# apple/ml-unigen

Measured on AMD Instinct MI355X. Metric: train-step samples/s (1.5B, 256^2 img), higher is better.
Workload: dtype bf16

## Files before the change

include/unigen_hip.h:

```cpp
#ifndef UNIGEN_HIP_H
#define UNIGEN_HIP_H

#include <stdint.h>
#include <hip/hip_runtime_api.h>

#ifdef __cplusplus
extern "C" {
#endif

#define UG_ABI_VERSION 7

const char* ug_last_error(void);
int ug_abi_version(void);

typedef struct ug_handle ug_handle;
int ug_create(ug_handle** out);
int ug_destroy(ug_handle* h);

#define UG_EPI_BF16 0
#define UG_EPI_F32 1
#define UG_EPI_RESID 2
int ug_gemm_bf16(const ug_handle* h, const void* A, int64_t lda, int a_kmajor, const void* B, int64_t ldb, int b_kmajor,
                 void* C, int64_t ldc, int64_t M, int64_t N, int64_t K, int epilogue, const void* bias,
                 const float* resid, int64_t ldr, int beta, const float* alpha_dev, int policy, hipStream_t stream);
// ... 42 lines not shown
#define UG_MASK_I64 2
#define UG_MASK_BOOL 3
int ug_attn_mask_compress(const void* mask, int mask_dtype, int64_t stride_b, int64_t stride_row,
                          uint64_t* bits, uint8_t* tileany, int64_t B, int64_t L, int* err_flag,
                          hipStream_t stream);
int ug_attn_mask_causal(const uint8_t* key_valid , uint64_t* bits, uint8_t* tileany,
                        int64_t B, int64_t L, hipStream_t stream);
int ug_attn_fwd(const void* q, const void* k, const void* v, int64_t ldq, void* o,
                int64_t ldo, float* lse, const uint64_t* bits, const uint8_t* tileany, int64_t B, int64_t L,
                int64_t Lp, int H, int HKV, int head_dim, float scale, hipStream_t stream);
int ug_attn_bwd(const void* q, const void* k, const void* v, int64_t ldq,
                const void* o, const void* dout, int64_t ldo, const float* lse,
                float* delta, void* dq, void* dk, void* dv, int64_t ldg, const uint64_t* bits,
                const uint8_t* tileany, int64_t B, int64_t L, int64_t Lp, int H, int HKV, int head_dim,
                float scale, float* dkv_ws, const float* rope_cos, const float* rope_sin, float* dbias_qkv, hipStream_t stream);

int ug_kv_store(const void* qkv, int64_t ldq, int64_t k_col, int64_t v_col, void* cache_k, void* cache_v,
                int64_t rows, int64_t L, int HKV, int head_dim, int64_t Tmax, const int* pos_dev, int pos_host,
                hipStream_t stream);
int ug_rope_at(void* qkv, const float* cos_tab, const float* sin_tab, int64_t rows, int64_t ldq, int nheads,
               int head_dim, const int* pos_dev, int64_t max_pos, hipStream_t stream);
int ug_attn_decode(const void* q, int64_t ldq, const void* cache_k, const void* cache_v, const uint8_t* key_valid,
                   void* o, int64_t ldo, int64_t rows, int H, int HKV, int head_dim, int64_t Tmax,
                   const int* len_dev, float scale, hipStream_t stream);
int ug_gemv_bf16(const void* x, int64_t ldx, int64_t R, const void* W, int64_t ldw, float* acc, int64_t acc_stride_r,
                 int64_t acc_stride_n, int64_t N, int64_t K, hipStream_t stream);
int ug_decode_finish_resid_norm(float* acc, int64_t ldacc, float* x, const float* w, void* xn, int64_t rows, int64_t cols,
                                float eps, int* pos_inc, int* len_inc, hipStream_t stream);
int ug_decode_gemv(const void* x, int64_t ldx, int64_t R, const void* W, int64_t ldw, float* acc, int64_t ldacc, int64_t N,
                   int64_t K, float* zero0, int64_t n0, float* zero1, int64_t n1, float* ss_zero, hipStream_t stream);
// ... 170 lines not shown
```

ml-unigen_amd/csrc/attention.hip:

```cpp
#include "common.h"
#include "unigen_hip.h"
#include "vmem_asm.h"
#include <stdlib.h>

namespace {

constexpr int HD = 128;
constexpr int RM_LD = 144;
constexpr int RM_BYTES = 64 * RM_LD * 2;
typedef __attribute__((ext_vector_type(4))) short s16x4_t;

template <typename T> __device__ __forceinline__ bool mask_attend(T v, int* err);
template <> __device__ __forceinline__ bool mask_attend<float>(float v, int* err) {
  if (v == 0.f) return true;
  if (!(v <= -1e9f) && err) atomicOr(err, 2);
  return false;
}
template <> __device__ __forceinline__ bool mask_attend<bf16_t>(bf16_t v, int* err) { return mask_attend<float>(bf2f(v), err); }
template <> __device__ __forceinline__ bool mask_attend<int64_t>(int64_t v, int* err) {
  if (v == 0) return true;
  if (v > -1000000000LL && err) atomicOr(err, 2);
  return false;
}
template <> __device__ __forceinline__ bool mask_attend<uint8_t>(uint8_t v, int*) { return v != 0; }
// ... 151 lines not shown

struct AttnArgs {
  const bf16_t* q; const bf16_t* k; const bf16_t* v;
  bf16_t* o; const bf16_t* dout;
  bf16_t* dq; bf16_t* dk; bf16_t* dv;
  float* dkv_ws;
  float* lse; const float* delta;
  const uint64_t* bits; const uint8_t* tileany;
  int64_t ldq, ldo, ldg;
  int B, L, Lp, nW, H, HKV;
  float scale;
  const float* rope_cos; const float* rope_sin; float* dbias;
  int order;
  int dkv_heads;
  int ablate;
};

__device__ __forceinline__ void rope_bwd_pair(float& g1, float& g2, float c, float s) {
#pragma clang fp contract(off)
  const float x1 = bf2f(f2bf(g1)), x2 = bf2f(f2bf(g2));
  const float a1 = x1 * c, a2 = x2 * c;
  const float b1 = x2 * s, b2 = x1 * s;
  g1 = a1 + b1; g2 = a2 - b2;
}
template <int N>
__device__ __forceinline__ void halve_sum(float (&x)[64], int lane, int m) {
  const bool up = (lane & m) != 0;
#pragma unroll
  for (int i = 0; i < N / 2; ++i) {
    const float lo = x[i], hi = x[i + N / 2];
// ... 748 lines not shown
  return ((row & 3) << 2) | ((0x78 >> (m * 2)) & 3);
}
__device__ __forceinline__ bf16x8_t frag16(const char* tile, int rb, int ks, int lane) {
  const int row = rb * 16 + (lane & 15);
  return *reinterpret_cast<const bf16x8_t*>(tile + row * 256 + (((ks * 4 + (lane >> 4)) ^ swz16b(row)) << 4));
}
__device__ __forceinline__ bf16x8_t frag16_tr(const char* tile, int rb, int jp, int lane) {
  const int i16 = lane & 15, g = lane >> 4;
  const int row = jp * 32 + g * 4 + (i16 >> 2);
  const char* p0 = tile + row * 256 + (((rb * 2 + ((i16 & 3) >> 1)) ^ swz16b(row)) << 4) + (i16 & 1) * 8;
  const s16x4_t lo = __builtin_amdgcn_ds_read_tr16_b64_v4i16((__attribute__((address_space(3))) s16x4_t*)p0);
  const s16x4_t hi = __builtin_amdgcn_ds_read_tr16_b64_v4i16((__attribute__((address_space(3))) s16x4_t*)(p0 + 16 * 256));
  return __builtin_shufflevector(lo, hi, 0, 1, 2, 3, 4, 5, 6, 7);
}

__global__ __launch_bounds__(256, 2) void attn_bwd_dkv_dma_kernel(AttnArgs p) {
  __shared__ __attribute__((aligned(16))) char ring[2 * 2 * T32_BYTES];
  __shared__ __attribute__((aligned(16))) float lse_s[2][64], dl_s[2][64];
  __shared__ __attribute__((aligned(16))) uint64_t word_s[2][64];
  const int tid = threadIdx.x, lane = tid & 63, g = lane >> 4;
  const int wave = __builtin_amdgcn_readfirstlane(tid >> 6);
  const int grp = p.H / p.HKV;
  const int HPW = p.dkv_heads;
  const WgCoord wc = wg_coord((int)blockIdx.x, p.nW, p.H / HPW, p.HKV, p.B, false, p.order != 0);
  if (!wc.ok) return;
  const int t = wc.tile, b = wc.b, h0 = wc.h * HPW, hk = h0 / grp;
  const int krow = t * 64 + wave * 16 + (lane & 15);
  const int krow_c = min(krow, p.L - 1);
  const bf16_t* kseq = p.k + (int64_t)b * p.L * p.ldq + hk * HD;
  const bf16_t* vseq = p.v + (int64_t)b * p.L * p.ldq + hk * HD;
// ... 56 lines not shown
  bool r_in = false;
  auto fetch_rows = [&](int qt) {
    const int qr = qt * 64 + lane;
    const int qc = min(qr, p.L - 1);
    r_lse = p.lse[((int64_t)b * p.H + h) * p.L + qc];
    r_dl = p.delta[((int64_t)b * p.H + h) * p.L + qc];
    r_word = p.bits[((int64_t)b * p.L + qc) * p.nW + t];
    r_in = qr < p.L;
  };

  int qt = next_visible(0);
  int hleft = qt < p.nW ? HPW - 1 : 0;
  if (qt < p.nW) { stage(qt, 0); if (wave == 0) fetch_rows(qt); }
#pragma unroll
  for (int ks = 0; ks < 4; ++ks) { tie(kf[ks]); tie(vf[ks]); }
  for (int it = 0; qt < p.nW; ++it) {
    int qn = next_visible(qt + 1);
    const int slot = it & 1;
    wait_vm<0>();
    if (wave == 0) {
      tie(r_lse); tie(r_dl); tie(r_word);
      lse_s[slot][lane] = r_lse * 1.4426950408889634f;
      dl_s[slot][lane] = r_dl * p.scale;
      word_s[slot][lane] = r_in ? r_word : 0ull;
    }
    asm volatile("s_waitcnt lgkmcnt(0)" ::: "memory");
    asm volatile("s_barrier" ::: "memory");
    if (qn >= p.nW && hleft > 0) {
      --hleft; ++h;
      qseq += HD; doseq += HD;
      qn = next_visible(0);
    }
    if (qn < p.nW) { stage(qn, slot ^ 1); if (wave == 0) fetch_rows(qn); }
// ... 9 lines not shown
        dp = __builtin_amdgcn_mfma_f32_16x16x32_bf16(frag16(Ds, j, ks, lane), vf[ks], dp, 0, 0, 0);
      }
      const f32x4_t ls = *reinterpret_cast<const f32x4_t*>(&lse_s[slot][j * 16 + g * 4]);
      const f32x4_t dl4 = *reinterpret_cast<const f32x4_t*>(&dl_s[slot][j * 16 + g * 4]);
#pragma unroll
      for (int r = 0; r < 4; ++r) {
        const int ql = j * 16 + g * 4 + r;
        const bool on = (word_s[slot][ql] >> kbit) & 1ull;
        const float e = on ? __builtin_amdgcn_exp2f(__builtin_fmaf(sc[r], c1, -ls[r])) : 0.f;
        pr[j][r] = e;
        ds[j][r] = e * __builtin_fmaf(dp[r], p.scale, -dl4[r]);
      }
    }
    const bf16x8_t pf0 = pack_p(pr[0], pr[1]), pf1 = pack_p(pr[2], pr[3]);
    const bf16x8_t sf0 = pack_p(ds[0], ds[1]), sf1 = pack_p(ds[2], ds[3]);
#pragma unroll
    for (int d = 0; d < 8; ++d) {
      dvt[d] = __builtin_amdgcn_mfma_f32_16x16x32_bf16(frag16_tr(Ds, d, 0, lane), pf0, dvt[d], 0, 0, 0);
      dkt[d] = __builtin_amdgcn_mfma_f32_16x16x32_bf16(frag16_tr(Qs, d, 0, lane), sf0, dkt[d], 0, 0, 0);
    }
#pragma unroll
    for (int d = 0; d < 8; ++d) {
      dvt[d] = __builtin_amdgcn_mfma_f32_16x16x32_bf16(frag16_tr(Ds, d, 1, lane), pf1, dvt[d], 0, 0, 0);
      dkt[d] = __builtin_amdgcn_mfma_f32_16x16x32_bf16(frag16_tr(Qs, d, 1, lane), sf1, dkt[d], 0, 0, 0);
    }
    qt = qn;
  }
  __syncthreads();
  float* tw = reinterpret_cast<float*>(ring) + wave * (16 * 132);
  const int ldws = 2 * p.HKV * HD;
// ... 4 lines not shown
#pragma unroll
      for (int r = 0; r < 4; ++r) tw[(lane & 15) * 132 + d * 16 + g * 4 + r] = pass == 0 ? dkt[d][r] : dvt[d][r];
    __builtin_amdgcn_wave_barrier();
    asm volatile("s_waitcnt lgkmcnt(0)" ::: "memory");
#pragma unroll
    for (int i = 0; i < 16; ++i) {
      const int kr = t * 64 + wave * 16 + i;
      if (kr < p.L) {
        float* dst = p.dkv_ws + ((int64_t)b * p.L + kr) * ldws + (pass * p.HKV + hk) * HD;
        atomicAdd(dst + lane, tw[i * 132 + lane]);
        atomicAdd(dst + 64 + lane, tw[i * 132 + 64 + lane]);
      }
    }
    __builtin_amdgcn_wave_barrier();
    asm volatile("s_waitcnt lgkmcnt(0)" ::: "memory");
  }
}

__global__ __launch_bounds__(256) void dkv_finish_rope_kernel(float* __restrict__ ws, bf16_t* __restrict__ dk, bf16_t* __restrict__ dv,
                                                              int64_t ldg, int64_t tokens, int L, int HKV,
                                                              const float* __restrict__ cs, const float* __restrict__ sn,
                                                              float* __restrict__ dbias_k, float* __restrict__ dbias_v,
                                                              int rows_per_block) {
  __shared__ float red[256 * 16];
  const int per_row = HKV * 16;
  const int slot = threadIdx.x / per_row, nslots = 256 / per_row;
  const int hk = (threadIdx.x % per_row) >> 4, c4 = threadIdx.x & 15;
  const int kvw = HKV * HD;
  float sum[16];
#pragma unroll
// ... 67 lines not shown
    float4* src = reinterpret_cast<float4*>(ws + row * 2 * kvw + c);
    const float4 v = *src;
    *src = make_float4(0.f, 0.f, 0.f, 0.f);
    uint2 w; w.x = pack_bf2(v.x, v.y); w.y = pack_bf2(v.z, v.w);
    bf16_t* dst = c < kvw ? dk + row * ldg + c : dv + row * ldg + (c - kvw);
    *reinterpret_cast<uint2*>(dst) = w;
  }
}

int check_common(const char* fn, int64_t B, int64_t L, int64_t Lp, int H, int HKV, int hd, int64_t ldq) {
  UG_REQUIRE(B > 0 && L > 0, "%s: empty batch", fn);
  UG_REQUIRE(hd == HD, "%s: head_dim %d unsupported (this build is specialised for 128)", fn, hd);
  UG_REQUIRE(H % HKV == 0, "%s: H=%d not a multiple of HKV=%d", fn, H, HKV);
  UG_REQUIRE(Lp % 64 == 0 && Lp >= L, "%s: Lp=%ld must be a multiple of 64 and >= L", fn, (long)Lp);
  UG_REQUIRE(ldq % 8 == 0, "%s: row stride must be a multiple of 8 elements", fn);
  return UG_OK;
}

}

extern "C" int ug_attn_mask_compress(const void* mask, int mask_dtype, int64_t stride_b, int64_t stride_row,
                                     uint64_t* bits, uint8_t* tileany, int64_t B, int64_t L, int* err_flag,
                                     hipStream_t st) {
  UG_REQUIRE(B > 0 && L > 0 && mask && bits && tileany, "ug_attn_mask_compress: bad args");
  const int nW = (int)((L + 63) / 64);
  const int64_t nwaves = B * L * nW;
  dim3 grid((unsigned)((nwaves + 3) / 4)), block(256);
  switch (mask_dtype) {
    case UG_MASK_F32: hipLaunchKernelGGL(mask_compress_kernel<float>, grid, block, 0, st, (const float*)mask, stride_b, stride_row, bits, (int)B, (int)L, nW, err_flag); break;
    case UG_MASK_BF16: hipLaunchKernelGGL(mask_compress_kernel<bf16_t>, grid, block, 0, st, (const bf16_t*)mask, stride_b, stride_row, bits, (int)B, (int)L, nW, err_flag); break;
// ... 70 lines not shown
  if (int rc = check_common("ug_attn_bwd", B, L, Lp, H, HKV, head_dim, ldq)) return rc;
  UG_REQUIRE((rope_cos == nullptr) == (rope_sin == nullptr) && (!rope_cos || (ug_aligned16(rope_cos) && ug_aligned16(rope_sin))),
             "ug_attn_bwd: rope_cos / rope_sin come together, 16-byte aligned");
  UG_REQUIRE(ug_aligned16(dkv_ws), "ug_attn_bwd: workspace alignment");
  UG_REQUIRE(ug_aligned16(q) && ug_aligned16(k) && ug_aligned16(v) && ug_aligned16(dout) && ldo % 8 == 0 && ldg % 4 == 0,
             "ug_attn_bwd: alignment");
  AttnArgs a{};
  a.q = (const bf16_t*)q; a.k = (const bf16_t*)k; a.v = (const bf16_t*)v;
  a.dout = (const bf16_t*)dout; a.lse = const_cast<float*>(lse); a.delta = delta;
  a.o = const_cast<bf16_t*>((const bf16_t*)o);
  a.dq = (bf16_t*)dq; a.dk = (bf16_t*)dk; a.dv = (bf16_t*)dv; a.dkv_ws = dkv_ws;
  a.bits = bits; a.tileany = tileany;
  a.ldq = ldq; a.ldo = ldo; a.ldg = ldg; a.B = (int)B; a.L = (int)L; a.Lp = (int)Lp; a.nW = (int)((L + 63) / 64);
  a.H = H; a.HKV = HKV; a.scale = scale;
  { static const int abl = [] { const char* e = getenv("UNIGEN_ATTN_ABLATE"); return e ? atoi(e) : 0; }(); a.ablate = abl; }
  static const int use32 = [] { const char* e = getenv("UNIGEN_ATTN_DQ32"); return e ? atoi(e) : 1; }();
  static const int fuse = [] { const char* e = getenv("UNIGEN_ATTN_BWD_FUSE_ROPE"); return e ? atoi(e) : 1; }();
  const int64_t tokens = B * L;
  auto rope_pass = [&](void* x, int nheads) -> int { return rope_cos ? ug_rope(x, rope_cos, rope_sin, tokens, L, ldg, nheads, HD, 1, st) : UG_OK; };
  auto colsum_pass = [&](const void* x, float* out, int cols) -> int { return dbias ? ug_colsum_bf16(x, ldg, out, tokens, cols, st) : UG_OK; };
  static const int ord = [] { const char* e = getenv("UNIGEN_ATTN_ORDER"); return e ? atoi(e) : 1; }();
  a.order = (ord >> 1) & 1;
  if (use32 && L >= 256 && L <= 4096 && (int64_t)((L + 127) / 128) * H * B >= 512) {
    if (fuse) { a.rope_cos = rope_cos; a.rope_sin = rope_sin; a.dbias = dbias; }
    hipLaunchKernelGGL(attn_bwd_dq32_kernel<4>, dim3(wg_grid((L + 127) / 128, H, HKV, B)), dim3(256), 0, st, a);
    UG_CHECK_LAUNCH("ug_attn_bwd(dq)");
    if (!fuse) { if (int rc = rope_pass(dq, H)) return rc; if (int rc = colsum_pass(dq, dbias, H * HD)) return rc; }
  } else {
    hipLaunchKernelGGL(attn_bwd_dq_kernel, dim3(wg_grid(a.nW, H, HKV, B)), dim3(256), 0, st, a);
    UG_CHECK_LAUNCH("ug_attn_bwd(dq)");
    if (int rc = rope_pass(dq, H)) return rc;
    if (int rc = colsum_pass(dq, dbias, H * HD)) return rc;
  }
  a.rope_cos = a.rope_sin = nullptr; a.dbias = nullptr;
  float* dbias_k = dbias ? dbias + H * HD : nullptr;
  float* dbias_v = dbias ? dbias + (H + HKV) * HD : nullptr;
  if (dkv_ws) {
    static const int dma = [] { const char* e = getenv("UNIGEN_ATTN_DKV_DMA"); return e ? atoi(e) : 1; }();
    a.order = (ord >> 2) & 1;
    static const int hpw_env = [] { const char* e = getenv("UNIGEN_ATTN_DKV_HEADS"); return e ? atoi(e) : 2; }();
    static const int hpw_min_wgs = [] { const char* e = getenv("UNIGEN_ATTN_DKV_MIN_WGS"); return e ? atoi(e) : 1024; }();
    a.dkv_heads = (hpw_env >= 1 && (H / HKV) % hpw_env == 0 && (int64_t)a.nW * (H / hpw_env) * B >= hpw_min_wgs) ? hpw_env : 1;
    if (dma && L <= 4096) hipLaunchKernelGGL(attn_bwd_dkv_dma_kernel, dim3(wg_grid(a.nW, H / a.dkv_heads, HKV, B)), dim3(256), 0, st, a);
    else hipLaunchKernelGGL(attn_bwd_dkv_kernel<true>, dim3(wg_grid(a.nW, H, HKV, B)), dim3(256), 0, st, a);
    UG_CHECK_LAUNCH("ug_attn_bwd(dkv split)");
    if (fuse && (rope_cos || dbias) && HKV <= 16 && (HKV & (HKV - 1)) == 0) {
      static const int fin_wgs = [] { const char* e = getenv("UNIGEN_ATTN_FINISH_WGS"); return e ? atoi(e) : 128; }();
      const int rpb = (int)((tokens + fin_wgs - 1) / fin_wgs < 8 ? 8 : (tokens + fin_wgs - 1) / fin_wgs);
      hipLaunchKernelGGL(dkv_finish_rope_kernel, dim3((unsigned)((tokens + rpb - 1) / rpb)), dim3(256), 0, st, dkv_ws, a.dk, a.dv, ldg,
                         tokens, (int)L, HKV, rope_cos, rope_sin, dbias_k, dbias_v, rpb);
      UG_CHECK_LAUNCH("ug_attn_bwd(dkv finish + rope)");
      return UG_OK;
    }
    const int64_t total = B * L * (2 * HKV * HD / 4);
    int64_t gsz = (total + 255) / 256; if (gsz > 4096) gsz = 4096;
    hipLaunchKernelGGL(dkv_finish_kernel, dim3((unsigned)gsz), dim3(256), 0, st, dkv_ws, a.dk, a.dv, ldg, B * L, HKV * HD);
    UG_CHECK_LAUNCH("ug_attn_bwd(dkv finish)");
  } else {
    hipLaunchKernelGGL(attn_bwd_dkv_kernel<false>, dim3(wg_grid(a.nW, HKV, HKV, B)), dim3(256), 0, st, a);
    UG_CHECK_LAUNCH("ug_attn_bwd(dkv)");
  }
  if (int rc = rope_pass(dk, HKV)) return rc;
  if (int rc = colsum_pass(dk, dbias_k, HKV * HD)) return rc;
  if (int rc = colsum_pass(dv, dbias_v, HKV * HD)) return rc;
  return UG_OK;
}
```

ml-unigen_amd/unigen_hip/lib.py:

```python
import ctypes
import os
import subprocess

_HERE = os.path.dirname(os.path.abspath(__file__))
CSRC_DIR = os.path.normpath(os.path.join(_HERE, "..", "csrc"))
LIB_PATH = os.environ.get("UNIGEN_HIP_LIB") or os.path.join(CSRC_DIR, "libunigen_hip.so")

ABI_VERSION = 7
P = ctypes.c_void_p
I64 = ctypes.c_int64
I32 = ctypes.c_int
F32 = ctypes.c_float

SIGNATURES = {
    "ug_abi_version": [],
    "ug_create": [P],
    "ug_destroy": [P],
    "ug_gemm_bf16": [P, P, I64, I32, P, I64, I32, P, I64, I64, I64, I64, I32, P, P, I64, I32, P, I32, P],
    "ug_gemm_bf16_qkv_rope": [P, P, I64, P, I64, P, P, I64, I64, I64, I64, P, P, I64, I64, I32, P],
    "ug_gemm_bf16_swiglu_bwd": [P, P, I64, P, I64, P, I64, P, I64, I64, I64, I64, P],
    "ug_gemm_bf16_swiglu": [P, P, I64, P, I64, P, I64, P, I64, I64, I64, I64, P],
    "ug_cast_f32_bf16": [P, P, I64, P],
    "ug_rmsnorm_fwd": [P, P, P, P, I64, I64, F32, I32, P],
    "ug_rmsnorm_bwd": [P, P, P, P, P, P, P, I64, I64, P],
    "ug_rope": [P, P, P, I64, I64, I64, I32, I32, I32, P],
    "ug_swiglu_fwd": [P, P, I64, I64, P],
    "ug_swiglu_bwd": [P, P, P, I64, I64, P],
    "ug_gelu": [P, P, P, I64, P],
    "ug_embed_fwd": [P, P, P, I64, I64, I64, P, P],
    "ug_embed_bwd": [P, P, P, I64, I64, I64, P],
    "ug_embed_bwd_sorted": [P, P, P, P, I64, I64, I64, F32, P],
    "ug_gather_rows_bf16": [P, I64, P, P, I64, I64, I64, I32, P],
    "ug_colsum_bf16": [P, I64, P, I64, I64, P],
    "ug_attn_mask_compress": [P, I32, I64, I64, P, P, I64, I64, P, P],
    "ug_attn_mask_causal": [P, P, P, I64, I64, P],
    "ug_attn_fwd": [P, P, P, I64, P, I64, P, P, P, I64, I64, I64, I32, I32, I32, F32, P],
    "ug_attn_bwd": [P, P, P, I64, P, P, I64, P, P, P, P, P, I64, P, P, I64, I64, I64, I32, I32, I32, F32, P, P, P, P, P],
    "ug_kv_store": [P, I64, I64, I64, P, P, I64, I64, I32, I32, I64, P, I32, P],
    "ug_rope_at": [P, P, P, I64, I64, I32, I32, P, I64, P],
    "ug_attn_decode": [P, I64, P, P, P, P, I64, I64, I32, I32, I32, I64, P, F32, P],
    "ug_gemv_bf16": [P, I64, I64, P, I64, P, I64, I64, I64, I64, P],
    "ug_decode_gemv": [P, I64, I64, P, I64, P, I64, I64, I64, P, I64, P, I64, P, P],
    "ug_decode_gemv_resid_norm": [P, P, I64, P, P, P, I64, P, I64, P, I64, I64, I64, P, I64, P, I64, P, P],
    "ug_decode_gemv_swiglu": [P, I64, P, F32, I64, I64, P, I64, P, I64, I64, I64, P, I64, P, I64, P, P],
    "ug_gemm_set_fused_tile_height": [I32],
    "ug_attn_decode_fused": [P, I64, P, F32, I64, P, P, P, P, P, P, P, P, I64, I64, I32, I32, I32, I64, I64, F32, P],
    "ug_decode_finish_resid_norm": [P, I64, P, P, P, I64, I64, F32, P, P, P],
    "ug_decode_sw_supported": [I64, I64, I64, I32],
    "ug_decode_sw_kblock": [P, I64, I64, P, I64, P, I64, I64, I64, P, I64, P, I64, P, P],
    "ug_decode_sw_resid": [P, I64, I64, P, I64, I64, I64, P, P],
    "ug_decode_sw_gate_up": [P, P, I64, P, P, F32, I64, I64, P, I64, I64, P, I64, P],
    "ug_decode_sw_head": [P, P, I64, P, P, F32, I64, I64, P, I64, I64, P, I64, P, P, P],
# ... 54 lines not shown
    "ug_nchw_to_nhwc": [P, P, I64, I32, I64, I32, P],
    "ug_nhwc_to_nchw": [P, P, I64, I32, I64, I32, P],
    "ug_lfq_pack": [P, I64, P, I64, I32, P],
    "ug_lfq_unpack": [P, P, I64, I32, P, P],
    "ug_probe_layouts": [P, I64, P],
}

_lib = None

PROFILE = None


def family_of(name):
    if name.startswith("ug_gemm_bf16"):
        return "gemm"
    if name in ("ug_attn_fwd", "ug_attn_bwd"):
        return "attention"
    if name.startswith(("ug_conv", "ug_groupnorm", "ug_amax", "ug_lfq", "ug_nchw", "ug_nhwc", "ug_gemm_f32", "ug_softmax_rows", "ug_linear_",
                        "ug_layernorm", "ug_siglip")):
        return "tokenizer_and_towers"
    if name == "ug_adamw_flat":
        return "adamw"
    return "elementwise"


def _profiled(name, fn):
    fam = family_of(name)

    def call(*args):
        prof = PROFILE
        if prof is None:
# ... 67 lines not shown
```

ml-unigen_amd/unigen_hip/ops.py:

```python
import ctypes
import math
import torch

from . import lib as _l

UG_EPI_BF16, UG_EPI_F32, UG_EPI_RESID = 0, 1, 2
_MASK_DTYPES = {torch.float32: 0, torch.bfloat16: 1, torch.int64: 2, torch.bool: 3}


GEMM_PROFILE = None
GEMM_PROFILE_FUSED = None


def _stream():
    return torch.cuda.current_stream().cuda_stream


def _p(t):
    return 0 if t is None else t.data_ptr()


_HANDLES = {}
GEMM_POLICY = -1
UG_GEMM_NARROW_EPILOGUE, UG_GEMM_POLICY_AUTO_BITS = 0x100, 0xff
# ... 407 lines not shown
                                   _p(mb.tileany), B, L, Lp, H, HKV, hd, scale, _stream()), "ug_attn_fwd")
    return o, lse


_DKV_WS = {}


def _dkv_workspace(tokens, width, device):
    key = (device, tokens, width)
    if key not in _DKV_WS:
        _DKV_WS.clear()
        _DKV_WS[key] = torch.zeros((tokens, width), dtype=torch.float32, device=device)
    return _DKV_WS[key]


def attn_bwd(qkv, o, lse, dout, mb, H, HKV, hd, scale=None, split_heads=True, rope=None, dbias=None, out=None):
    B, L, Lp = mb.B, mb.L, mb.Lp
    scale = 1.0 / math.sqrt(hd) if scale is None else scale
    q = qkv[:, : H * hd]
    k = qkv[:, H * hd: (H + HKV) * hd]
    v = qkv[:, (H + HKV) * hd:]
    dqkv = torch.empty_like(qkv) if out is None else out
    dq = dqkv[:, : H * hd]
    dk = dqkv[:, H * hd: (H + HKV) * hd]
    dv = dqkv[:, (H + HKV) * hd:]
    delta = torch.empty((B, H, L), dtype=torch.float32, device=qkv.device)
    ws = _dkv_workspace(B * L, 2 * HKV * hd, qkv.device) if split_heads and H > HKV else None
    _l.check(_l.load().ug_attn_bwd(_p(q), _p(k), _p(v), qkv.stride(0), _p(o), _p(dout), o.stride(0),
                                   _p(lse), _p(delta), _p(dq), _p(dk), _p(dv), dqkv.stride(0), _p(mb.bits),
                                   _p(mb.tileany), B, L, Lp, H, HKV, hd, scale, _p(ws), _p(rope[0] if rope else None),
                                   _p(rope[1] if rope else None), _p(dbias), _stream()), "ug_attn_bwd")
    return dqkv


def kv_store(qkv, cache_k, cache_v, rows, L, H, HKV, hd, Tmax, pos_dev=None, pos_host=0):
    _l.check(_l.load().ug_kv_store(_p(qkv), qkv.stride(0), H * hd, (H + HKV) * hd, _p(cache_k), _p(cache_v), rows, L, HKV, hd,
                                   Tmax, _p(pos_dev), pos_host, _stream()), "ug_kv_store")


def rope_at_(qkv, cos, sin, nheads, hd, pos_dev):
    _l.check(_l.load().ug_rope_at(_p(qkv), _p(cos), _p(sin), qkv.shape[0], qkv.stride(0), nheads, hd, _p(pos_dev),
                                  cos.shape[0], _stream()), "ug_rope_at")
# ... 613 lines not shown
```

Baseline: 130.3.

## Hand off dS from dK/dV kernel to a dQ kernel instead of recomputing

Adds an attention backward route where the dK/dV kernel writes each bf16 dS tile to a global workspace. A new dQ kernel then streams K and dS tiles and does only the dS·K matmul, so it no longer recomputes QK^T, softmax and dP. A separate delta kernel is added, and the route is on by default for eligible GQA shapes. The cost is a workspace of up to 1 GiB (B·H·nW²·8KB) and the extra HBM traffic to write and re-read dS, and the dQ pass now has to run after dK/dV instead of alongside it.

```diff
diff --git a/include/unigen_hip.h b/include/unigen_hip.h
--- a/include/unigen_hip.h
+++ b/include/unigen_hip.h
@@ -80,6 +80,12 @@
                 float* delta, void* dq, void* dk, void* dv, int64_t ldg, const uint64_t* bits,
                 const uint8_t* tileany, int64_t B, int64_t L, int64_t Lp, int H, int HKV, int head_dim,
                 float scale, float* dkv_ws, const float* rope_cos, const float* rope_sin, float* dbias_qkv, hipStream_t stream);
+int ug_attn_bwd_handoff(const void* q, const void* k, const void* v, int64_t ldq,
+                        const void* o, const void* dout, int64_t ldo, const float* lse,
+                        float* delta, void* dq, void* dk, void* dv, int64_t ldg, const uint64_t* bits,
+                        const uint8_t* tileany, int64_t B, int64_t L, int64_t Lp, int H, int HKV, int head_dim,
+                        float scale, float* dkv_ws, const float* rope_cos, const float* rope_sin, float* dbias_qkv,
+                        void* ds_ws, int64_t ds_ws_bytes, int dkv_heads, hipStream_t stream);
 
 int ug_kv_store(const void* qkv, int64_t ldq, int64_t k_col, int64_t v_col, void* cache_k, void* cache_v,
                 int64_t rows, int64_t L, int HKV, int head_dim, int64_t Tmax, const int* pos_dev, int pos_host,
diff --git a/ml-unigen_amd/csrc/attention.hip b/ml-unigen_amd/csrc/attention.hip
--- a/ml-unigen_amd/csrc/attention.hip
+++ b/ml-unigen_amd/csrc/attention.hip
@@ -189,6 +189,8 @@
   int order;
   int dkv_heads;
   int ablate;
+  char* ds_ws;
+  int delta_lanes;
 };
 
 __device__ __forceinline__ void rope_bwd_pair(float& g1, float& g2, float c, float s) {
@@ -967,6 +969,8 @@
   return __builtin_shufflevector(lo, hi, 0, 1, 2, 3, 4, 5, 6, 7);
 }
 
+constexpr int DS_BLOCK = 64 * 64 * 2;
+template <bool HANDOFF>
 __global__ __launch_bounds__(256, 2) void attn_bwd_dkv_dma_kernel(AttnArgs p) {
   __shared__ __attribute__((aligned(16))) char ring[2 * 2 * T32_BYTES];
   __shared__ __attribute__((aligned(16))) float lse_s[2][64], dl_s[2][64];
@@ -1053,9 +1057,11 @@
   if (qt < p.nW) { stage(qt, 0); if (wave == 0) fetch_rows(qt); }
 #pragma unroll
   for (int ks = 0; ks < 4; ++ks) { tie(kf[ks]); tie(vf[ks]); }
+  const uint32_t dsoff = (uint32_t)(wave * 2048 + ((g * 16 + ((lane & 15) ^ (g << 2))) << 4));
   for (int it = 0; qt < p.nW; ++it) {
     int qn = next_visible(qt + 1);
     const int slot = it & 1;
+    const int hcur = h;
     wait_vm<0>();
     if (wave == 0) {
       tie(r_lse); tie(r_dl); tie(r_word);
@@ -1095,6 +1101,11 @@
     }
     const bf16x8_t pf0 = pack_p(pr[0], pr[1]), pf1 = pack_p(pr[2], pr[3]);
     const bf16x8_t sf0 = pack_p(ds[0], ds[1]), sf1 = pack_p(ds[2], ds[3]);
+    if constexpr (HANDOFF) {
+      char* blk = p.ds_ws + ((((int64_t)b * p.H + hcur) * p.nW + qt) * p.nW + t) * DS_BLOCK + dsoff;
+      *reinterpret_cast<bf16x8_t*>(blk) = sf0;
+      *reinterpret_cast<bf16x8_t*>(blk + 1024) = sf1;
+    }
 #pragma unroll
     for (int d = 0; d < 8; ++d) {
       dvt[d] = __builtin_amdgcn_mfma_f32_16x16x32_bf16(frag16_tr(Ds, d, 0, lane), pf0, dvt[d], 0, 0, 0);
@@ -1129,6 +1140,198 @@
     }
     __builtin_amdgcn_wave_barrier();
     asm volatile("s_waitcnt lgkmcnt(0)" ::: "memory");
+  }
+}
+
+
+template <int NP>
+__global__ __launch_bounds__(256) void attn_bwd_delta_kernel(AttnArgs p) {
+  const int64_t idx = (int64_t)blockIdx.x * 256 + threadIdx.x;
+  const int part = (int)(idx % NP);
+  const int64_t rh = idx / NP;
+  const int h = (int)(rh % p.H);
+  const int64_t row = min(rh / p.H, (int64_t)p.B * p.L - 1);
+  const bool in = rh / p.H < (int64_t)p.B * p.L;
+  const bf16_t* orow = p.o + row * p.ldo + h * HD;
+  const bf16_t* drow = p.dout + row * p.ldo + h * HD;
+  float dl = 0.f;
+#pragma unroll
+  for (int ks = 0; ks < 16 / NP; ++ks) {
+    const bf16x8_t dof = *reinterpret_cast<const bf16x8_t*>(drow + (ks * NP + part) * 8);
+    const bf16x8_t of = *reinterpret_cast<const bf16x8_t*>(orow + (ks * NP + part) * 8);
+#pragma unroll
+    for (int e = 0; e < 8; ++e) dl += bf2f((bf16_t)of[e]) * bf2f((bf16_t)dof[e]);
+  }
+  dl += __shfl_xor(dl, 1, 64);
+  if (NP == 4) dl += __shfl_xor(dl, 2, 64);
+  if (part == 0 && in) const_cast<float*>(p.delta)[((row / p.L) * p.H + h) * p.L + row % p.L] = dl;
+}
+
+__global__ __launch_bounds__(256, 2) void attn_bwd_dq_handoff_kernel(AttnArgs p) {
+  __shared__ __attribute__((aligned(16))) char ring[2 * 2 * T32_BYTES];
+  const int tid = threadIdx.x, lane = tid & 63;
+  const int wave = __builtin_amdgcn_readfirstlane(tid >> 6);
+  const int n = lane & 31, hh = lane >> 5, i16 = lane & 15, grp = (lane >> 4) & 1;
+  const WgCoord wc = wg_coord((int)blockIdx.x, (p.L + 127) / 128, p.H, p.HKV, p.B, true, p.order != 0);
+  if (!wc.ok) return;
+  const int qt = wc.tile, h = wc.h, b = wc.b;
+  const int hk = h / (p.H / p.HKV);
+  const int qrow = qt * 128 + wave * 32 + n;
+  const bool qlive = qrow < p.L;
+  const int qrow_c = min(qrow, p.L - 1);
+  const bf16_t* kseq = p.k + (int64_t)b * p.L * p.ldq + hk * HD;
+  const int qb0 = qt * 2;
+  const bool two = qb0 + 1 < p.nW;
+  uint64_t v0, v1;
+  {
+    bool a0 = false, a1 = false;
+    if (lane < p.nW) {
+      a0 = p.tileany[((int64_t)b * p.nW + qb0) * p.nW + lane];
+      if (two) a1 = p.tileany[((int64_t)b * p.nW + qb0 + 1) * p.nW + lane];
+    }
+    v0 = __ballot(a0);
+    v1 = __ballot(a1);
+  }
+  const uint64_t vis = v0 | v1, minem = (wave >> 1) ? v1 : v0;
+  auto next_visible = [&](int t) {
+    const uint64_t rest = t < 64 ? vis >> t : 0ull;
+    return rest ? t + __builtin_ctzll(rest) : p.nW;
+  };
+  uint32_t toff[4];
+#pragma unroll
+  for (int i = 0; i < 4; ++i) {
+    const int row = (i * 4 + wave) * 4 + (lane >> 4);
+    toff[i] = (uint32_t)(row * p.ldq + (((lane & 15) ^ swz16(row)) << 3)) * 2u;
+  }
+  const char* dsrow = p.ds_ws + (((int64_t)b * p.H + h) * p.nW + qb0) * p.nW * DS_BLOCK;
+  auto stage = [&](int t, int slot) {
+    char* base = ring + slot * 2 * T32_BYTES;
+    const uint64_t kb = (uint64_t)kseq + (int64_t)t * 64 * p.ldq * 2;
+    if (t * 64 + 64 <= p.L) {
+#pragma unroll
+      for (int i = 0; i < 4; ++i)
+        dma16(kb, toff[i], __builtin_amdgcn_readfirstlane(lds_addr_of(base + (i * 4 + wave) * 1024)));
+    } else {
+#pragma unroll
+      for (int i = 0; i < 4; ++i) {
+        const int inst = i * 4 + wave;
+        const int row = inst * 4 + (lane >> 4);
+        const uint32_t off = (uint32_t)((min(t * 64 + row, p.L - 1) - t * 64) * p.ldq + (((lane & 15) ^ swz16(row)) << 3)) * 2u;
+        dma16(kb, off, __builtin_amdgcn_readfirstlane(lds_addr_of(base + inst * 1024)));
+      }
+    }
+#pragma unroll
+    for (int u = 0; u < 2; ++u)
+      if ((u ? v1 >> t : v0 >> t) & 1ull) {
+        const uint64_t dbv = (uint64_t)dsrow + ((int64_t)u * p.nW + t) * DS_BLOCK;
+        const uint64_t db = ((uint64_t)(uint32_t)__builtin_amdgcn_readfirstlane((int)(dbv >> 32)) << 32) |
+                            (uint32_t)__builtin_amdgcn_readfirstlane((int)(uint32_t)dbv);
+#pragma unroll
+        for (int i = 0; i < 2; ++i) {
+          const int inst = i * 4 + wave;
+          dma16_nt(db + inst * 1024, (uint32_t)lane * 16u, __builtin_amdgcn_readfirstlane(lds_addr_of(base + T32_BYTES + u * DS_BLOCK + inst * 1024)));
+        }
+      }
+  };
+  int voff[4][2], doff[2];
+#pragma unroll
+  for (int e = 0; e < 2; ++e) {
+    const int key = 4 * hh + (i16 >> 2) + 8 * e;
+#pragma unroll
+    for (int d = 0; d < 4; ++d) {
+      const int chunk = d * 4 + grp * 2 + ((i16 & 3) >> 1);
+      voff[d][e] = key * 256 + ((chunk ^ swz16(key)) << 4) + (i16 & 1) * 8;
+    }
+    const int pc = i16 & 3;
+    doff[e] = (wave >> 1) * DS_BLOCK + (wave & 1) * 1024 + ((pc * 16 + (key ^ (pc << 2))) << 4) + grp * 8;
+  }
+  f32x16_t dqt[4];
+#pragma unroll
+  for (int d = 0; d < 4; ++d)
+#pragma unroll
+    for (int r = 0; r < 16; ++r) dqt[d][r] = 0.f;
+
+  int t = next_visible(0);
+  if (t < p.nW) stage(t, 0);
+  for (int it = 0; t < p.nW; ++it) {
+    const int tn = next_visible(t + 1);
+    wait_vm<0>();
+    asm volatile("s_barrier" ::: "memory");
+    if (tn < p.nW) stage(tn, (it + 1) & 1);
+    if ((minem >> t) & 1ull) {
+      const char* Ks = ring + (it & 1) * 2 * T32_BYTES;
+      const char* Ds = Ks + T32_BYTES;
+#pragma unroll
+      for (int kb = 0; kb < 2; ++kb)
+#pragma unroll
+        for (int j = 0; j < 2; ++j) {
+          const char* db_ = Ds + (kb * 2 + j) * 2048;
+          const s16x4_t slo = __builtin_amdgcn_ds_read_tr16_b64_v4i16((__attribute__((address_space(3))) s16x4_t*)(db_ + doff[0]));
+          const s16x4_t shi = __builtin_amdgcn_ds_read_tr16_b64_v4i16((__attribute__((address_space(3))) s16x4_t*)(db_ + doff[1]));
+          const bf16x8_t sf = __builtin_shufflevector(slo, shi, 0, 1, 2, 3, 4, 5, 6, 7);
+          const char* kb_ = Ks + kb * 8192 + j * 4096;
+#pragma unroll
+          for (int d = 0; d < 4; ++d) {
+            const s16x4_t lo = __builtin_amdgcn_ds_read_tr16_b64_v4i16((__attribute__((address_space(3))) s16x4_t*)(kb_ + voff[d][0]));
+            const s16x4_t hi = __builtin_amdgcn_ds_read_tr16_b64_v4i16((__attribute__((address_space(3))) s16x4_t*)(kb_ + voff[d][1]));
+            const bf16x8_t a = __builtin_shufflevector(lo, hi, 0, 1, 2, 3, 4, 5, 6, 7);
+            dqt[d] = __builtin_amdgcn_mfma_f32_32x32x16_bf16(__builtin_bit_cast(hwbf16x8_t, a), __builtin_bit_cast(hwbf16x8_t, sf),
+                                                             dqt[d], 0, 0, 0);
+          }
+        }
+    }
+    t = tn;
+  }
+  if (p.rope_cos) {
+#pragma unroll
+    for (int d = 0; d < 2; ++d)
+#pragma unroll
+      for (int q = 0; q < 4; ++q) {
+        const int col = d * 32 + q * 8 + hh * 4;
+        const float4 c = *reinterpret_cast<const float4*>(p.rope_cos + (int64_t)qrow_c * (HD / 2) + col);
+        const float4 sn = *reinterpret_cast<const float4*>(p.rope_sin + (int64_t)qrow_c * (HD / 2) + col);
+        const float cc[4] = {c.x, c.y, c.z, c.w}, ss[4] = {sn.x, sn.y, sn.z, sn.w};
+#pragma unroll
+        for (int e = 0; e < 4; ++e) {
+          float g1 = dqt[d][q * 4 + e], g2 = dqt[d + 2][q * 4 + e];
+          rope_bwd_pair(g1, g2, cc[e], ss[e]);
+          dqt[d][q * 4 + e] = g1; dqt[d + 2][q * 4 + e] = g2;
+        }
+      }
+  }
+  if (qlive) {
+    bf16_t* drow = p.dq + ((int64_t)b * p.L + qrow) * p.ldg + h * HD;
+#pragma unroll
+    for (int d = 0; d < 4; ++d)
+#pragma unroll
+      for (int q = 0; q < 4; ++q) {
+        uint2 w;
+        w.x = pack_bf2(dqt[d][q * 4 + 0], dqt[d][q * 4 + 1]);
+        w.y = pack_bf2(dqt[d][q * 4 + 2], dqt[d][q * 4 + 3]);
+        *reinterpret_cast<uint2*>(drow + d * 32 + q * 8 + hh * 4) = w;
+      }
+  }
+  if (p.dbias) {
+    float x[64];
+#pragma unroll
+    for (int d = 0; d < 4; ++d)
+#pragma unroll
+      for (int r = 0; r < 16; ++r) x[d * 16 + r] = qlive ? bf2f(f2bf(dqt[d][r])) : 0.f;
+    lanes32_colsum(x, lane);
+    __syncthreads();
+    float* red = reinterpret_cast<float*>(ring);
+#pragma unroll
+    for (int e = 0; e < 2; ++e) {
+      const int v = 2 * n + e, d = v >> 4, r = v & 15;
+      red[wave * HD + d * 32 + (r >> 2) * 8 + hh * 4 + (r & 3)] = x[e];
+    }
+    __syncthreads();
+    if (tid < HD) {
+      float s = 0.f;
+#pragma unroll
+      for (int w = 0; w < 4; ++w) s += red[w * HD + tid];
+      atomicAdd(p.dbias + h * HD + tid, s);
+    }
   }
 }
 
@@ -1226,6 +1429,40 @@
   UG_REQUIRE(H % HKV == 0, "%s: H=%d not a multiple of HKV=%d", fn, H, HKV);
   UG_REQUIRE(Lp % 64 == 0 && Lp >= L, "%s: Lp=%ld must be a multiple of 64 and >= L", fn, (long)Lp);
   UG_REQUIRE(ldq % 8 == 0, "%s: row stride must be a multiple of 8 elements", fn);
+  return UG_OK;
+}
+
+int env_dq32() { static const int v = [] { const char* e = getenv("UNIGEN_ATTN_DQ32"); return e ? atoi(e) : 1; }(); return v; }
+int env_fuse_rope() { static const int v = [] { const char* e = getenv("UNIGEN_ATTN_BWD_FUSE_ROPE"); return e ? atoi(e) : 1; }(); return v; }
+int env_order() { static const int v = [] { const char* e = getenv("UNIGEN_ATTN_ORDER"); return e ? atoi(e) : 1; }(); return v; }
+bool dq32_shape(int64_t B, int64_t L, int H) { return env_dq32() && L >= 256 && L <= 4096 && (int64_t)((L + 127) / 128) * H * B >= 512; }
+int dkv_heads_rule(int64_t B, int nW, int H, int HKV) {
+  static const int hpw_env = [] { const char* e = getenv("UNIGEN_ATTN_DKV_HEADS"); return e ? atoi(e) : 2; }();
+  static const int hpw_min_wgs = [] { const char* e = getenv("UNIGEN_ATTN_DKV_MIN_WGS"); return e ? atoi(e) : 1024; }();
+  return (hpw_env >= 1 && (H / HKV) % hpw_env == 0 && (int64_t)nW * (H / hpw_env) * B >= hpw_min_wgs) ? hpw_env : 1;
+}
+int finish_split_dkv(const AttnArgs& a, int64_t B, int64_t L, int H, int HKV, int64_t ldg, float* dkv_ws, const float* rope_cos,
+                     const float* rope_sin, float* dbias, hipStream_t st) {
+  const int64_t tokens = B * L;
+  float* dbias_k = dbias ? dbias + H * HD : nullptr;
+  float* dbias_v = dbias ? dbias + (H + HKV) * HD : nullptr;
+  if (env_fuse_rope() && (rope_cos || dbias) && HKV <= 16 && (HKV & (HKV - 1)) == 0) {
+    static const int fin_wgs = [] { const char* e = getenv("UNIGEN_ATTN_FINISH_WGS"); return e ? atoi(e) : 128; }();
+    const int rpb = (int)((tokens + fin_wgs - 1) / fin_wgs < 8 ? 8 : (tokens + fin_wgs - 1) / fin_wgs);
+    hipLaunchKernelGGL(dkv_finish_rope_kernel, dim3((unsigned)((tokens + rpb - 1) / rpb)), dim3(256), 0, st, dkv_ws, a.dk, a.dv, ldg,
+                       tokens, (int)L, HKV, rope_cos, rope_sin, dbias_k, dbias_v, rpb);
+    UG_CHECK_LAUNCH("ug_attn_bwd(dkv finish + rope)");
+    return UG_OK;
+  }
+  const int64_t total = B * L * (2 * HKV * HD / 4);
+  int64_t gsz = (total + 255) / 256; if (gsz > 4096) gsz = 4096;
+  hipLaunchKernelGGL(dkv_finish_kernel, dim3((unsigned)gsz), dim3(256), 0, st, dkv_ws, a.dk, a.dv, ldg, B * L, HKV * HD);
+  UG_CHECK_LAUNCH("ug_attn_bwd(dkv finish)");
+  if (rope_cos) if (int rc = ug_rope(a.dk, rope_cos, rope_sin, tokens, L, ldg, HKV, HD, 1, st)) return rc;
+  if (dbias) {
+    if (int rc = ug_colsum_bf16(a.dk, ldg, dbias_k, tokens, HKV * HD, st)) return rc;
+    if (int rc = ug_colsum_bf16(a.dv, ldg, dbias_v, tokens, HKV * HD, st)) return rc;
+  }
   return UG_OK;
 }
 
@@ -1326,14 +1563,13 @@
   a.ldq = ldq; a.ldo = ldo; a.ldg = ldg; a.B = (int)B; a.L = (int)L; a.Lp = (int)Lp; a.nW = (int)((L + 63) / 64);
   a.H = H; a.HKV = HKV; a.scale = scale;
   { static const int abl = [] { const char* e = getenv("UNIGEN_ATTN_ABLATE"); return e ? atoi(e) : 0; }(); a.ablate = abl; }
-  static const int use32 = [] { const char* e = getenv("UNIGEN_ATTN_DQ32"); return e ? atoi(e) : 1; }();
-  static const int fuse = [] { const char* e = getenv("UNIGEN_ATTN_BWD_FUSE_ROPE"); return e ? atoi(e) : 1; }();
+  const int fuse = env_fuse_rope();
   const int64_t tokens = B * L;
   auto rope_pass = [&](void* x, int nheads) -> int { return rope_cos ? ug_rope(x, rope_cos, rope_sin, tokens, L, ldg, nheads, HD, 1, st) : UG_OK; };
   auto colsum_pass = [&](const void* x, float* out, int cols) -> int { return dbias ? ug_colsum_bf16(x, ldg, out, tokens, cols, st) : UG_OK; };
-  static const int ord = [] { const char* e = getenv("UNIGEN_ATTN_ORDER"); return e ? atoi(e) : 1; }();
+  const int ord = env_order();
   a.order = (ord >> 1) & 1;
-  if (use32 && L >= 256 && L <= 4096 && (int64_t)((L + 127) / 128) * H * B >= 512) {
+  if (dq32_shape(B, L, H)) {
     if (fuse) { a.rope_cos = rope_cos; a.rope_sin = rope_sin; a.dbias = dbias; }
     hipLaunchKernelGGL(attn_bwd_dq32_kernel<4>, dim3(wg_grid((L + 127) / 128, H, HKV, B)), dim3(256), 0, st, a);
     UG_CHECK_LAUNCH("ug_attn_bwd(dq)");
@@ -1350,24 +1586,11 @@
   if (dkv_ws) {
     static const int dma = [] { const char* e = getenv("UNIGEN_ATTN_DKV_DMA"); return e ? atoi(e) : 1; }();
     a.order = (ord >> 2) & 1;
-    static const int hpw_env = [] { const char* e = getenv("UNIGEN_ATTN_DKV_HEADS"); return e ? atoi(e) : 2; }();
-    static const int hpw_min_wgs = [] { const char* e = getenv("UNIGEN_ATTN_DKV_MIN_WGS"); return e ? atoi(e) : 1024; }();
-    a.dkv_heads = (hpw_env >= 1 && (H / HKV) % hpw_env == 0 && (int64_t)a.nW * (H / hpw_env) * B >= hpw_min_wgs) ? hpw_env : 1;
-    if (dma && L <= 4096) hipLaunchKernelGGL(attn_bwd_dkv_dma_kernel, dim3(wg_grid(a.nW, H / a.dkv_heads, HKV, B)), dim3(256), 0, st, a);
+    a.dkv_heads = dkv_heads_rule(B, a.nW, H, HKV);
+    if (dma && L <= 4096) hipLaunchKernelGGL(attn_bwd_dkv_dma_kernel<false>, dim3(wg_grid(a.nW, H / a.dkv_heads, HKV, B)), dim3(256), 0, st, a);
     else hipLaunchKernelGGL(attn_bwd_dkv_kernel<true>, dim3(wg_grid(a.nW, H, HKV, B)), dim3(256), 0, st, a);
     UG_CHECK_LAUNCH("ug_attn_bwd(dkv split)");
-    if (fuse && (rope_cos || dbias) && HKV <= 16 && (HKV & (HKV - 1)) == 0) {
-      static const int fin_wgs = [] { const char* e = getenv("UNIGEN_ATTN_FINISH_WGS"); return e ? atoi(e) : 128; }();
-      const int rpb = (int)((tokens + fin_wgs - 1) / fin_wgs < 8 ? 8 : (tokens + fin_wgs - 1) / fin_wgs);
-      hipLaunchKernelGGL(dkv_finish_rope_kernel, dim3((unsigned)((tokens + rpb - 1) / rpb)), dim3(256), 0, st, dkv_ws, a.dk, a.dv, ldg,
-                         tokens, (int)L, HKV, rope_cos, rope_sin, dbias_k, dbias_v, rpb);
-      UG_CHECK_LAUNCH("ug_attn_bwd(dkv finish + rope)");
-      return UG_OK;
-    }
-    const int64_t total = B * L * (2 * HKV * HD / 4);
-    int64_t gsz = (total + 255) / 256; if (gsz > 4096) gsz = 4096;
-    hipLaunchKernelGGL(dkv_finish_kernel, dim3((unsigned)gsz), dim3(256), 0, st, dkv_ws, a.dk, a.dv, ldg, B * L, HKV * HD);
-    UG_CHECK_LAUNCH("ug_attn_bwd(dkv finish)");
+    return finish_split_dkv(a, B, L, H, HKV, ldg, dkv_ws, rope_cos, rope_sin, dbias, st);
   } else {
     hipLaunchKernelGGL(attn_bwd_dkv_kernel<false>, dim3(wg_grid(a.nW, HKV, HKV, B)), dim3(256), 0, st, a);
     UG_CHECK_LAUNCH("ug_attn_bwd(dkv)");
@@ -1377,3 +1600,57 @@
   if (int rc = colsum_pass(dv, dbias_v, HKV * HD)) return rc;
   return UG_OK;
 }
+
+extern "C" int ug_attn_bwd_handoff(const void* q, const void* k, const void* v, int64_t ldq,
+                                   const void* o, const void* dout, int64_t ldo, const float* lse,
+                                   float* delta, void* dq, void* dk, void* dv, int64_t ldg, const uint64_t* bits,
+                                   const uint8_t* tileany, int64_t B, int64_t L, int64_t Lp, int H, int HKV, int head_dim,
+                                   float scale, float* dkv_ws, const float* rope_cos, const float* rope_sin, float* dbias,
+                                   void* ds_ws, int64_t ds_ws_bytes, int dkv_heads, hipStream_t st) {
+  if (int rc = check_common("ug_attn_bwd_handoff", B, L, Lp, H, HKV, head_dim, ldq)) return rc;
+  UG_REQUIRE(L >= 256 && L <= 4096, "ug_attn_bwd_handoff: L=%ld outside [256, 4096] (use ug_attn_bwd)", (long)L);
+  UG_REQUIRE(H > HKV, "ug_attn_bwd_handoff: H == HKV has no split-head dK / dV kernel (use ug_attn_bwd)");
+  UG_REQUIRE(dkv_ws && ug_aligned16(dkv_ws), "ug_attn_bwd_handoff: the split-head workspace is required, 16-byte aligned");
+  UG_REQUIRE(q && k && v && o && dout && lse && delta && dq && dk && dv && bits && tileany, "ug_attn_bwd_handoff: null tensor");
+  UG_REQUIRE((rope_cos == nullptr) == (rope_sin == nullptr) && (!rope_cos || (ug_aligned16(rope_cos) && ug_aligned16(rope_sin))),
+             "ug_attn_bwd_handoff: rope_cos / rope_sin come together, 16-byte aligned");
+  UG_REQUIRE(ug_aligned16(q) && ug_aligned16(k) && ug_aligned16(v) && ug_aligned16(dout) && ug_aligned16(o) && ldo % 8 == 0 && ldg % 4 == 0 &&
+             ((uintptr_t)dq & 7) == 0, "ug_attn_bwd_handoff: alignment");
+  const int nW = (int)((L + 63) / 64);
+  const int64_t need = B * H * nW * nW * DS_BLOCK;
+  UG_REQUIRE(ds_ws && ug_aligned16(ds_ws) && ds_ws_bytes >= need, "ug_attn_bwd_handoff: dS workspace of %ld bytes, %ld needed (16-byte aligned)",
+             (long)ds_ws_bytes, (long)need);
+  UG_REQUIRE(dkv_heads >= 0 && dkv_heads <= 2 && (dkv_heads == 0 || (H / HKV) % dkv_heads == 0),
+             "ug_attn_bwd_handoff: dkv_heads=%d must be 0 (the rule of ug_attn_bwd), 1 or 2 and divide H / HKV", dkv_heads);
+  AttnArgs a{};
+  a.q = (const bf16_t*)q; a.k = (const bf16_t*)k; a.v = (const bf16_t*)v;
+  a.dout = (const bf16_t*)dout; a.lse = const_cast<float*>(lse); a.delta = delta;
+  a.o = const_cast<bf16_t*>((const bf16_t*)o);
+  a.dq = (bf16_t*)dq; a.dk = (bf16_t*)dk; a.dv = (bf16_t*)dv; a.dkv_ws = dkv_ws; a.ds_ws = (char*)ds_ws;
+  a.bits = bits; a.tileany = tileany;
+  a.ldq = ldq; a.ldo = ldo; a.ldg = ldg; a.B = (int)B; a.L = (int)L; a.Lp = (int)Lp; a.nW = nW;
+  a.H = H; a.HKV = HKV; a.scale = scale;
+  const int fuse = env_fuse_rope(), ord = env_order();
+  const int64_t tokens = B * L;
+  {
+    const int np = dq32_shape(B, L, H) ? 2 : 4;
+    const unsigned grid = (unsigned)((tokens * H * np + 255) / 256);
+    if (np == 2) hipLaunchKernelGGL(attn_bwd_delta_kernel<2>, dim3(grid), dim3(256), 0, st, a);
+    else hipLaunchKernelGGL(attn_bwd_delta_kernel<4>, dim3(grid), dim3(256), 0, st, a);
+    UG_CHECK_LAUNCH("ug_attn_bwd_handoff(delta)");
+  }
+  a.order = (ord >> 2) & 1;
+  a.dkv_heads = dkv_heads ? dkv_heads : dkv_heads_rule(B, nW, H, HKV);
+  hipLaunchKernelGGL(attn_bwd_dkv_dma_kernel<true>, dim3(wg_grid(nW, H / a.dkv_heads, HKV, B)), dim3(256), 0, st, a);
+  UG_CHECK_LAUNCH("ug_attn_bwd_handoff(dkv + dS)");
+  if (int rc = finish_split_dkv(a, B, L, H, HKV, ldg, dkv_ws, rope_cos, rope_sin, dbias, st)) return rc;
+  a.order = (ord >> 1) & 1;
+  if (fuse) { a.rope_cos = rope_cos; a.rope_sin = rope_sin; a.dbias = dbias; }
+  hipLaunchKernelGGL(attn_bwd_dq_handoff_kernel, dim3(wg_grid((L + 127) / 128, H, HKV, B)), dim3(256), 0, st, a);
+  UG_CHECK_LAUNCH("ug_attn_bwd_handoff(dq)");
+  if (!fuse) {
+    if (rope_cos) if (int rc = ug_rope(dq, rope_cos, rope_sin, tokens, L, ldg, H, HD, 1, st)) return rc;
+    if (dbias) if (int rc = ug_colsum_bf16(dq, ldg, dbias, tokens, H * HD, st)) return rc;
+  }
+  return UG_OK;
+}
diff --git a/ml-unigen_amd/unigen_hip/lib.py b/ml-unigen_amd/unigen_hip/lib.py
--- a/ml-unigen_amd/unigen_hip/lib.py
+++ b/ml-unigen_amd/unigen_hip/lib.py
@@ -36,6 +36,7 @@
     "ug_attn_mask_causal": [P, P, P, I64, I64, P],
     "ug_attn_fwd": [P, P, P, I64, P, I64, P, P, P, I64, I64, I64, I32, I32, I32, F32, P],
     "ug_attn_bwd": [P, P, P, I64, P, P, I64, P, P, P, P, P, I64, P, P, I64, I64, I64, I32, I32, I32, F32, P, P, P, P, P],
+    "ug_attn_bwd_handoff": [P, P, P, I64, P, P, I64, P, P, P, P, P, I64, P, P, I64, I64, I64, I32, I32, I32, F32, P, P, P, P, P, I64, I32, P],
     "ug_kv_store": [P, I64, I64, I64, P, P, I64, I64, I32, I32, I64, P, I32, P],
     "ug_rope_at": [P, P, P, I64, I64, I32, I32, P, I64, P],
     "ug_attn_decode": [P, I64, P, P, P, P, I64, I64, I32, I32, I32, I64, P, F32, P],
@@ -120,7 +121,7 @@
 def family_of(name):
     if name.startswith("ug_gemm_bf16"):
         return "gemm"
-    if name in ("ug_attn_fwd", "ug_attn_bwd"):
+    if name in ("ug_attn_fwd", "ug_attn_bwd", "ug_attn_bwd_handoff"):
         return "attention"
     if name.startswith(("ug_conv", "ug_groupnorm", "ug_amax", "ug_lfq", "ug_nchw", "ug_nhwc", "ug_gemm_f32", "ug_softmax_rows", "ug_linear_",
                         "ug_layernorm", "ug_siglip")):
diff --git a/ml-unigen_amd/unigen_hip/ops.py b/ml-unigen_amd/unigen_hip/ops.py
--- a/ml-unigen_amd/unigen_hip/ops.py
+++ b/ml-unigen_amd/unigen_hip/ops.py
@@ -1,4 +1,5 @@
 import ctypes
+import os
 import math
 import torch
 
@@ -445,7 +446,45 @@
     return _DKV_WS[key]
 
 
-def attn_bwd(qkv, o, lse, dout, mb, H, HKV, hd, scale=None, split_heads=True, rope=None, dbias=None, out=None):
+_DS_WS = {}
+DS_WS_CAP = 1 << 30
+HANDOFF_DEFAULT = True
+
+
+def _ds_workspace(nbytes, device):
+    key = (device, nbytes)
+    if key not in _DS_WS:
+        _DS_WS.clear()
+        _DS_WS[key] = torch.empty(nbytes, dtype=torch.uint8, device=device)
+    return _DS_WS[key]
+
+
+def attn_bwd_handoff_bytes(B, L, H):
+    nW = (L + 63) // 64
+    return B * H * nW * nW * 8192
+
+
+def attn_bwd_handoff_eligible(B, L, H, HKV, split_heads=True):
+    return bool(split_heads) and H > HKV and 256 <= L <= 4096
+
+
+def _attn_bwd_route(route, B, L, H, HKV, split_heads):
+    if route not in (None, "recompute", "handoff"):
+        raise ValueError(f"attn_bwd: route={route!r} (None, 'recompute' or 'handoff')")
+    ok = attn_bwd_handoff_eligible(B, L, H, HKV, split_heads)
+    if route == "handoff" and not ok:
+        raise ValueError(f"attn_bwd: route='handoff' needs the split-head workspace, H > HKV and 256 <= L <= 4096 "
+                         f"(got B={B} L={L} H={H} HKV={HKV} split_heads={split_heads})")
+    if route is not None:
+        return route
+    env = os.environ.get("UNIGEN_ATTN_BWD_HANDOFF")
+    want = HANDOFF_DEFAULT if env is None else env not in ("", "0")
+    measured = ((L + 127) // 128) * H * B >= 512
+    return "handoff" if want and ok and measured and attn_bwd_handoff_bytes(B, L, H) <= DS_WS_CAP else "recompute"
+
+
+def attn_bwd(qkv, o, lse, dout, mb, H, HKV, hd, scale=None, split_heads=True, rope=None, dbias=None, out=None, route=None,
+             dkv_heads=0, delta_out=None):
     B, L, Lp = mb.B, mb.L, mb.Lp
     scale = 1.0 / math.sqrt(hd) if scale is None else scale
     q = qkv[:, : H * hd]
@@ -455,8 +494,17 @@
     dq = dqkv[:, : H * hd]
     dk = dqkv[:, H * hd: (H + HKV) * hd]
     dv = dqkv[:, (H + HKV) * hd:]
-    delta = torch.empty((B, H, L), dtype=torch.float32, device=qkv.device)
+    delta = torch.empty((B, H, L), dtype=torch.float32, device=qkv.device) if delta_out is None else delta_out
     ws = _dkv_workspace(B * L, 2 * HKV * hd, qkv.device) if split_heads and H > HKV else None
+    if _attn_bwd_route(route, B, L, H, HKV, split_heads) == "handoff":
+        nbytes = attn_bwd_handoff_bytes(B, L, H)
+        ds = _ds_workspace(nbytes, qkv.device)
+        _l.check(_l.load().ug_attn_bwd_handoff(_p(q), _p(k), _p(v), qkv.stride(0), _p(o), _p(dout), o.stride(0),
+                                               _p(lse), _p(delta), _p(dq), _p(dk), _p(dv), dqkv.stride(0), _p(mb.bits),
+                                               _p(mb.tileany), B, L, Lp, H, HKV, hd, scale, _p(ws), _p(rope[0] if rope else None),
+                                               _p(rope[1] if rope else None), _p(dbias), _p(ds), nbytes, int(dkv_heads), _stream()),
+                 "ug_attn_bwd_handoff")
+        return dqkv
     _l.check(_l.load().ug_attn_bwd(_p(q), _p(k), _p(v), qkv.stride(0), _p(o), _p(dout), o.stride(0),
                                    _p(lse), _p(delta), _p(dq), _p(dk), _p(dv), dqkv.stride(0), _p(mb.bits),
                                    _p(mb.tileany), B, L, Lp, H, HKV, hd, scale, _p(ws), _p(rope[0] if rope else None),
```

Measured after the change: 131.2, median of 6. About the same (+0.7%).
